# Xiaoming-Zhao/PointNav-VO

Hardware: AMD Instinct MI355X
Metric: RGB-D frame-pair VO inferences/s @341x192 (higher is better)
Workload: dtype f32

## Files before the change

### pointnav-vo_amd/csrc/stem_rs.hip

```cpp
#include <type_traits>

#include "stem_tile.h"

namespace pnvo {

namespace {
constexpr int RS_BUF = XCHG_BYTES;
constexpr int RS_PB_OFF = 2 * RS_BUF;
constexpr int RS_RED_OFF = RS_PB_OFF + 8 * 16 * 33 * 4;
constexpr int RS_ETAB_OFF = RS_RED_OFF + 4 * 2 * 32 * 2 * 4;
constexpr int RS_TRASH_OFF = RS_ETAB_OFF + 64;
constexpr int RS_LDS = RS_TRASH_OFF + 64;
static_assert(RS_BUF >= PATCH_BYTES, "patch must fit its buffer");
static_assert(RS_LDS <= 160 * 1024, "LDS budget");
#define PNVO_INL __attribute__((always_inline))
template <int N, int I = 0, class F>
__device__ __forceinline__ void static_for(F &&f) {
  if constexpr (I < N) {
    f(std::integral_constant<int, I>{});
    static_for<N, I + 1>(f);
  }
}
#ifndef PNVO_RS_LAGD
#define PNVO_RS_LAGD 3
#endif
#ifndef PNVO_RS_LAGP
#define PNVO_RS_LAGP 3
#endif
#ifndef PNVO_RS_GDS
#define PNVO_RS_GDS 2
#endif
#ifndef PNVO_RS_GVM
#define PNVO_RS_GVM 1
#endif
#ifndef PNVO_RS_GVA
#define PNVO_RS_GVA 4
#endif
#ifndef PNVO_RS_A1AHEAD
#define PNVO_RS_A1AHEAD 0
#endif
#ifndef PNVO_RS_MERGE
#define PNVO_RS_MERGE 1
#endif
#ifndef PNVO_RS_MIN_TILES
#define PNVO_RS_MIN_TILES 4
#endif
#ifndef PNVO_RS_NPIN
#define PNVO_RS_NPIN 10
#endif
#ifndef PNVO_RS_ABL
#define PNVO_RS_ABL 0
#endif
}

template <int PIECES, bool POOL, bool RAW, bool FAST = false>
__global__ __launch_bounds__(256) __attribute__((amdgpu_waves_per_eu(1, 1))) void stem_rs_kernel(const StemMXArgs p) {
  static_assert(PIECES == 2 || (PIECES == 1 && !POOL && !FAST), "float16 pieces, or the bf16 dual stem with raw output");
  constexpr bool H = PIECES == 2;
  constexpr int NTL = H ? 1 : 2;
  constexpr int NFT = H ? 5 : 4;
  constexpr bool A1AHEAD = H && PNVO_RS_A1AHEAD;
  constexpr int LAGP = PNVO_RS_LAGP, LAGD = PNVO_RS_LAGD;
  constexpr int GROW = PW * 5;
  extern __shared__ __attribute__((aligned(16))) unsigned char lds[];
  const int tid = threadIdx.x;
  const int lane = tid & 63;
  const int wave = __builtin_amdgcn_readfirstlane(tid >> 6);
  float *red = reinterpret_cast<float *>(lds + RS_RED_OFF);
  float *pb = reinterpret_cast<float *>(lds + RS_PB_OFF);
  float *etab = reinterpret_cast<float *>(lds + RS_ETAB_OFF);

  const int ntiles = p.B * p.tiles_x * p.tiles_y;
  const int chunk = (ntiles + 7) >> 3;
  const int per = (int)gridDim.x >> 3;
  const int t_first = (int)(blockIdx.x & 7) * chunk + (int)(blockIdx.x >> 3);
  const int t_end = min(((int)(blockIdx.x & 7) + 1) * chunk, ntiles);
  if (t_first >= t_end) return;
  const int nit = (t_end - t_first + per - 1) / per;
  const bool prof = p.prof != nullptr;
  unsigned long long pc[4] = {0, 0, 0, 0};
  auto now = [&]() PNVO_INL -> unsigned long long { return prof ? __builtin_readcyclecounter() : 0ull; };
  if (RAW && tid < 12) etab[tid] = p.edges[tid];

  unsigned pmeta[4];
#pragma unroll
  for (int r = 0; r < 4; ++r) {
    const int pix = min(r * 256 + tid, NPIX - 1);
    const int py = pix / PW, px = pix - py * PW;
    pmeta[r] = (unsigned)(py * ROW + (px & 1) * PAR + (px >> 1) * PITCH) | ((unsigned)px << 16) | ((unsigned)py << 22);
  }
  const bool haslast = tid < NPIX - 3 * 256;
  unsigned gm[RAW ? 1 : 3];
  if (!RAW) {
#pragma unroll
    for (int sr = 0; sr < 3; ++sr) {
      const int g = sr * 64 + lane;
      const bool ex = g < GROW;
      const int gg = ex ? g : 0;
      const int px = gg / 5, c = gg - px * 5;
      gm[sr] = (unsigned)((px & 1) * PAR + (px >> 1) * PITCH + c * 8) | ((unsigned)px << 16) | (ex ? 0x80000000u : 0u);
    }
  }
  const unsigned lane16 = (unsigned)lane * 16u;
  const float *zp = p.zero_page;
  const long fpix = (long)p.H * p.W;

  f32x4 vr4[4], gdd[21];
  f32x2 vr2[4], vd[4], vt[4];
  unsigned rgbw[4][2];
  float dv[4][2];
  unsigned pflag[4];
  unsigned lowbits = 0, bad_depth = 0;
  constexpr unsigned OOB = 0x80000000u;
  int shi = 0, swi = 0;
  int st_n = 0, st_ty = 0, st_tx = 0;
  __amdgpu_buffer_rsrc_t r_rgb, r_d, r_dd, r_t;
  auto rsrc = [&](const void *base, long off, long bytes) PNVO_INL {
    return __builtin_amdgcn_make_buffer_rsrc(const_cast<char *>(base ? reinterpret_cast<const char *>(base) + off : reinterpret_cast<const char *>(zp)),
                                             0, base ? (unsigned)bytes : 0u, 0x00020000);
  };
  const int per_n = per / (p.tiles_x * p.tiles_y), per_r = per % (p.tiles_x * p.tiles_y), per_y = per_r / p.tiles_x, per_x = per_r % p.tiles_x;
  auto set_stage_coords = [&](int sn_i, int ty, int tx) PNVO_INL {
    const long sn = sn_i;
    shi = 2 * ty * TH - 3;
    swi = 2 * tx * TW - 3;
    st_n = sn_i;
    st_ty = ty;
    st_tx = tx;
    if (RAW) {
      r_rgb = rsrc(p.raw_rgb, sn * fpix * 6, fpix * 6);
      r_d = rsrc(p.raw_depth, sn * fpix * 8, fpix * 8);
      r_dd = rsrc(nullptr, 0, 0);
    } else {
      r_rgb = rsrc(p.src[0], sn * fpix * 24, fpix * 24);
      r_d = rsrc(p.src[1], sn * fpix * 8, fpix * 8);
      r_dd = rsrc(p.src[2], sn * fpix * 80, fpix * 80);
    }
    r_t = rsrc(p.src[3], sn * fpix * 8, fpix * 8);
  };
  auto stage_next_tile = [&](bool advance) PNVO_INL {
    int tx = st_tx + (advance ? per_x : 0);
    const int cx = tx >= p.tiles_x ? 1 : 0;
    tx -= cx * p.tiles_x;
    int ty = st_ty + (advance ? per_y + cx : 0);
    const int cy = ty >= p.tiles_y ? 1 : 0;
    ty -= cy * p.tiles_y;
    set_stage_coords(st_n + (advance ? per_n + cy : 0), ty, tx);
  };
  auto set_stage_tile = [&](int t) PNVO_INL {
    const int tx = t % p.tiles_x;
    t /= p.tiles_x;
    const int ty = t % p.tiles_y;
    const long sn = t / p.tiles_y;
    shi = 2 * ty * TH - 3;
    swi = 2 * tx * TW - 3;
    st_n = (int)sn;
    st_ty = ty;
    st_tx = tx;
    if (RAW) {
      r_rgb = rsrc(p.raw_rgb, sn * fpix * 6, fpix * 6);
      r_d = rsrc(p.raw_depth, sn * fpix * 8, fpix * 8);
      r_dd = rsrc(nullptr, 0, 0);
    } else {
      r_rgb = rsrc(p.src[0], sn * fpix * 24, fpix * 24);
      r_d = rsrc(p.src[1], sn * fpix * 8, fpix * 8);
      r_dd = rsrc(p.src[2], sn * fpix * 80, fpix * 80);
    }
    r_t = rsrc(p.src[3], sn * fpix * 8, fpix * 8);
  };
  auto opaque = [&](unsigned v) PNVO_INL {
    asm volatile("" : "+v"(v));
    return v;
  };
  auto load_px = [&](int r, bool exists) PNVO_INL {
    const unsigned pm = opaque(pmeta[r]);
    const int hi = shi + (int)(pm >> 22), wi = swi + (int)((pm >> 16) & 0x3fu);
    const bool in = (int)exists & (int)((unsigned)hi < (unsigned)p.H) & (int)((unsigned)wi < (unsigned)p.W);
    const unsigned e = (unsigned)(hi * p.W + wi);
    pflag[r] = (in ? 1u : 0u) | (e > 0u ? 2u : 0u);
    if (RAW) {
#pragma unroll
      for (int f = 0; f < 2; ++f) {
        const unsigned li = (unsigned)f * (unsigned)fpix + e;
        const unsigned boff = 3u * li - ((f > 0 || e > 0u) ? 1u : 0u);
        rgbw[r][f] = __builtin_amdgcn_raw_buffer_load_b32(r_rgb, in ? boff : OOB, 0, 0);
        dv[r][f] = __builtin_bit_cast(float, __builtin_amdgcn_raw_buffer_load_b32(r_d, in ? li * 4u : OOB, 0, 0));
      }
      vt[r] = __builtin_bit_cast(f32x2, __builtin_amdgcn_raw_buffer_load_b64(r_t, in ? e * 8u : OOB, 0, 0));
    } else {
      const unsigned o24 = in ? e * 24u : OOB, o8 = in ? e * 8u : OOB;
      const f32x2 q0 = __builtin_bit_cast(f32x2, __builtin_amdgcn_raw_buffer_load_b64(r_rgb, o24, 0, 0));
      const f32x2 q1 = __builtin_bit_cast(f32x2, __builtin_amdgcn_raw_buffer_load_b64(r_rgb, o24 + 8u, 0, 0));
      vr4[r] = f32x4{q0[0], q0[1], q1[0], q1[1]};
      vr2[r] = __builtin_bit_cast(f32x2, __builtin_amdgcn_raw_buffer_load_b64(r_rgb, o24 + 16u, 0, 0));
      vd[r] = __builtin_bit_cast(f32x2, __builtin_amdgcn_raw_buffer_load_b64(r_d, o8, 0, 0));
      vt[r] = __builtin_bit_cast(f32x2, __builtin_amdgcn_raw_buffer_load_b64(r_t, o8, 0, 0));
    }
  };
  unsigned wrgb[3] = {0u, 0u, 0u};
  constexpr float RGBS = H ? 0.00390625f : 1.f;
  constexpr unsigned ONE2 = H ? 0x3c003c00u : 0x3f803f80u;
  constexpr unsigned short ONE1 = H ? 0x3c00 : 0x3f80;
  auto store_px = [&](int r, unsigned buf, bool exists, int part) PNVO_INL {
    if (part != 2) {
      if (RAW) {
        const unsigned x0 = (pflag[r] & 2u) ? rgbw[r][0] >> 8 : rgbw[r][0], x1 = rgbw[r][1] >> 8;
        const float pr = (float)(x0 & 0xffu), pg = (float)((x0 >> 8) & 0xffu), pbl = (float)((x0 >> 16) & 0xffu);
        const float cr = (float)(x1 & 0xffu), cg = (float)((x1 >> 8) & 0xffu), cb = (float)((x1 >> 16) & 0xffu);
        wrgb[0] = pack_pair<H>(pr * RGBS, pg * RGBS);
        wrgb[1] = pack_pair<H>(pbl * RGBS, cr * RGBS);
        wrgb[2] = pack_pair<H>(cg * RGBS, cb * RGBS);
      } else {
        wrgb[0] = pack_pair<H>(vr4[r][0] * RGBS, vr4[r][1] * RGBS);
        wrgb[1] = pack_pair<H>(vr4[r][2] * RGBS, vr4[r][3] * RGBS);
        wrgb[2] = pack_pair<H>(vr2[r][0] * RGBS, vr2[r][1] * RGBS);
        const float f0 = vr4[r][0], f1 = vr4[r][1], f2 = vr4[r][2], f3 = vr4[r][3], f4 = vr2[r][0], f5 = vr2[r][1];
        lowbits |= __builtin_bit_cast(unsigned, f0) | __builtin_bit_cast(unsigned, f1);
        lowbits |= __builtin_bit_cast(unsigned, f2) | __builtin_bit_cast(unsigned, f3);
        lowbits |= __builtin_bit_cast(unsigned, f4) | __builtin_bit_cast(unsigned, f5);
      }
    }
    if (part == 1) return;
    float d0, d1;
    int bidx[2] = {0, 0};
    unsigned bok[2] = {0u, 0u};
    const bool in = (pflag[r] & 1u) != 0u;
    if (RAW) {
      const bool use_d = (p.raw_flags & 1) != 0;
#pragma unroll
      for (int f = 0; f < 2; ++f) {
        const float d = dv[r][f];
        int g = (int)(d * 10.0f);
        g = min(max(g, 0), 9);
        const float lo = etab[g], hi = etab[g + 1];
        bidx[f] = g - (d < lo ? 1 : 0) + (((d >= hi) & (g < 9)) ? 1 : 0);
        bok[f] = ((d >= 0.f) & (d <= 1.f)) ? 1u : 0u;
        bad_depth |= (pflag[r] & 1u) & (bok[f] ^ 1u);
      }
      d0 = use_d ? dv[r][0] : 0.f;
      d1 = use_d ? dv[r][1] : 0.f;
    } else {
      d0 = vd[r][0];
      d1 = vd[r][1];
    }
    const unsigned w13 = pack_pair<H>(d0, d1), w14 = pack_pair<H>(vt[r][0], vt[r][1]), w15 = in ? ONE2 : 0u;
    const unsigned base = buf + (opaque(pmeta[r]) & 0xffffu);
    constexpr unsigned TR = (unsigned)RS_TRASH_OFF;
    if (RAW) {
      *reinterpret_cast<u32x4 *>(lds + (exists ? base : TR)) = u32x4{0u, 0u, 0u, 0u};
      *reinterpret_cast<u32x4 *>(lds + (exists ? base + 16u : TR)) = u32x4{0u, 0u, 0u, 0u};
      *reinterpret_cast<u32x4 *>(lds + (exists ? base + 32u : TR)) = u32x4{0u, 0u, wrgb[0], wrgb[1]};
      *reinterpret_cast<u32x4 *>(lds + (exists ? base + 48u : TR)) = u32x4{wrgb[2], w13, w14, w15};
      const bool dd = (p.raw_flags & 2) != 0 && in && exists;
      *reinterpret_cast<unsigned short *>(lds + ((dd && bok[0]) ? base + 2u * (unsigned)bidx[0] : TR)) = ONE1;
      *reinterpret_cast<unsigned short *>(lds + ((dd && bok[1]) ? base + 20u + 2u * (unsigned)bidx[1] : TR)) = ONE1;
    } else {
      *reinterpret_cast<u32x2 *>(lds + (exists ? base + 40u : TR)) = u32x2{wrgb[0], wrgb[1]};
      *reinterpret_cast<u32x4 *>(lds + (exists ? base + 48u : TR)) = u32x4{wrgb[2], w13, w14, w15};
    }
    if (H) {
      const f16x2 hd = __builtin_bit_cast(f16x2, w13), ht = __builtin_bit_cast(f16x2, w14);
      const unsigned md = pack_f16(d0 - (float)hd[0], d1 - (float)hd[1]);
      const unsigned mt = pack_f16(vt[r][0] - (float)ht[0], vt[r][1] - (float)ht[1]);
      *reinterpret_cast<u32x4 *>(lds + (exists ? base + 64u : TR)) = u32x4{md, mt, 0u, 0u};
    }
  };
  unsigned ddv[3], ddl[3];
  auto set_dd_tile = [&](unsigned buf) PNVO_INL {
    if (RAW) return;
#pragma unroll
    for (int sr = 0; sr < 3; ++sr) {
      const unsigned g = opaque(gm[sr]);
      const int wi = swi + (int)((g >> 16) & 0x3fu);
      const bool ok = (int)((int)g < 0) & (int)((unsigned)wi < (unsigned)p.W);
      ddv[sr] = ok ? (unsigned)((shi * p.W + swi) * 80 + sr * 1024) + lane16 : OOB;
      ddl[sr] = buf + ((int)g < 0 ? (g & 0xffffu) : (unsigned)(2 * PAR));
    }
  };
  auto load_dd = [&](int slot, int row, int sr) PNVO_INL {
    gdd[slot] = __builtin_bit_cast(f32x4, __builtin_amdgcn_raw_buffer_load_b128(r_dd, ddv[sr] + (unsigned)(row * p.W * 80), 0, 0));
  };
  auto store_dd = [&](int slot, int row, int sr) PNVO_INL {
    const f32x4 v = gdd[slot];
    lowbits |= __builtin_bit_cast(unsigned, v[0]) | __builtin_bit_cast(unsigned, v[1]);
    lowbits |= __builtin_bit_cast(unsigned, v[2]) | __builtin_bit_cast(unsigned, v[3]);
    *reinterpret_cast<u32x2 *>(lds + ddl[sr] + row * ROW) = u32x2{pack_pair<H>(v[0], v[1]), pack_pair<H>(v[2], v[3])};
  };

  const int arr = (lane & 31) >> 4, ac = lane & 15, ah = lane >> 5;
  const unsigned baseA0 = (unsigned)(2 * arr * ROW + ac * PITCH + ah * 16);
  const unsigned baseX0 = (unsigned)(2 * arr * ROW + ac * PITCH + 64);
  const int rr16 = lane >> 5;
  const float oscale = !H ? 1.f : p.oscale_ptr != nullptr ? *p.oscale_ptr : p.oscale;
  const int co = p.y_coff[0] + (lane & 31);
  const float sgn = POOL ? (p.pool_gamma[co] < 0.f ? -1.f : 1.f) : 1.f;

  auto body = [&](auto wv_c) PNVO_INL {
    constexpr int WV = decltype(wv_c)::value;
    constexpr int NROWS = FAST ? (WV == 1 ? 6 : 5) : WV == 3 ? 0 : 7;
    constexpr int DPT = FAST ? 2 : 3, PX0 = FAST ? 1 : 0, PXS = FAST ? 3 : 2;
    auto px_store_tap = [](int i) constexpr { return i >= LAGP + PX0 && (i - LAGP - PX0) % PXS == 0 && (i - LAGP - PX0) / PXS < 3; };
    auto dd_row = [](int j) constexpr { return FAST ? (j < 5 ? WV + 4 * j : 20) : WV + 3 * j; };
    constexpr int RD = RAW ? 0 : 3 * NROWS;
    constexpr int NT = (WV == 3 && !FAST) ? 13 : 12;
    auto tap_of = [](int i) constexpr { return i < 12 ? WV + 4 * i : 48; };
    auto tap_off = [](int t) constexpr { return (t / 7) * ROW + ((t % 7) & 1) * PAR + ((t % 7) >> 1) * PITCH; };

    __syncthreads();
    set_stage_tile(t_first);
    set_dd_tile(0u);
#pragma unroll
    for (int r = 0; r < 3; ++r) load_px(r, true);
    if (WV == 0) load_px(3, haslast);
#pragma unroll
    for (int q = 0; q < RD; ++q) load_dd(q, dd_row(q / 3), q % 3);
#pragma unroll
    for (int r = 0; r < 3; ++r) store_px(r, 0u, true, 0);
    if (WV == 0) store_px(3, 0u, haslast, 0);
#pragma unroll
    for (int q = 0; q < RD; ++q) store_dd(q, dd_row(q / 3), q % 3);
    __syncthreads();

    u32x4 bres[NT][4];
    u32x2 bxr[(H && !FAST) ? NT : 1];
    u32x4 bxs[FAST ? 3 : 1], b48[FAST ? 4 : 1];
    u32x2 b48x = {0u, 0u};
    {
      const u32x4 *wp = reinterpret_cast<const u32x4 *>(p.wpk) + lane;
#pragma unroll
      for (int i = 0; i < NT; ++i) {
#pragma unroll
        for (int f = 0; f < 4; ++f) bres[i][f] = wp[(tap_of(i) * NFT + f) * 64];
        if (H && !FAST) bxr[i] = *reinterpret_cast<const u32x2 *>(wp + (tap_of(i) * NFT + 4) * 64);
      }
      if (FAST) {
        const u32x4 *wq = reinterpret_cast<const u32x4 *>(p.wpk) + (lane & 31);
        const bool kh1 = lane >= 32;
#pragma unroll
        for (int g = 0; g < 3; ++g) {
          const u32x2 lo = *reinterpret_cast<const u32x2 *>(wq + ((kh1 ? tap_of(4 * g + 2) : tap_of(4 * g)) * NFT + 4) * 64);
          const u32x2 hi = *reinterpret_cast<const u32x2 *>(wq + ((kh1 ? tap_of(4 * g + 3) : tap_of(4 * g + 1)) * NFT + 4) * 64);
          bxs[g] = u32x4{lo[0], lo[1], hi[0], hi[1]};
        }
#pragma unroll
        for (int f = 0; f < 4; ++f) b48[f] = wp[(48 * NFT + f) * 64];
        b48x = *reinterpret_cast<const u32x2 *>(wp + (48 * NFT + 4) * 64);
      }
      constexpr int NPIN = H ? PNVO_RS_NPIN : 7;
#pragma unroll
      for (int i = 0; i < (NT < NPIN ? NT : NPIN); ++i) {
#pragma unroll
        for (int f = 0; f < 4; ++f) asm volatile("" : "+a"(bres[i][f]));
        if (H && !FAST) asm volatile("" : "+a"(bxr[i]));
      }
      if (FAST) {
#pragma unroll
        for (int g = 0; g < 3; ++g) asm volatile("" : "+a"(bxs[g]));
      }
    }

    int e_n = 0, e_ho0 = 0, e_wo0 = 0, e_slot = 0;
    bool e_valid = false;
    unsigned ebuf = 0u;
    f32x4 xq[4], tq4;
    float s1 = 0.f, s2 = 0.f, cm[8], pl[6], rs9[3];
    f32x2 rsv[4];
    int rr16v = 0, lc = 0, colv = 0;
    auto epi_begin = [&]() PNVO_INL {
      rr16v = (int)opaque((unsigned)rr16);
      lc = (int)opaque((unsigned)(lane & 31));
      colv = p.Wo - e_wo0 - 4 * rr16v;
      s1 = 0.f;
      s2 = 0.f;
    };
    auto XAl = [&](int rq) PNVO_INL {
#pragma unroll
      for (int s4 = 0; s4 < 4; ++s4)
        xq[s4] = *reinterpret_cast<const f32x4 *>(lds + ebuf + (((WV * 4 + s4) * 4 + rq) * 64 + lane) * 16);
    };
    auto XAs = [&]() PNVO_INL {
#pragma unroll
      for (int e = 0; e < 4; ++e) tq4[e] = (((xq[0][e] + xq[1][e]) + xq[2][e]) + xq[3][e]) * oscale;
    };
    auto XB = [&](int rq) PNVO_INL {
      const bool rowok = e_ho0 + 2 * WV + (rq >> 1) < p.Ho;
#pragma unroll
      for (int e = 0; e < 4; ++e) {
        const int colc = e + 8 * (rq & 1);
        const bool ok = (int)rowok & (int)(colc < colv);
        const float v = ok ? tq4[e] : 0.f;
        pb[((2 * WV + (rq >> 1)) * 16 + colc + 4 * rr16v) * 33 + lc] = ok ? sgn * tq4[e] : -__builtin_inff();
        s1 += v;
        s2 = __builtin_fmaf(v, v, s2);
      }
    };
    auto XC = [&]() PNVO_INL {
      s1 += __shfl_xor(s1, 32);
      s2 += __shfl_xor(s2, 32);
      *reinterpret_cast<f32x2 *>(&red[(WV * 32 + lc) * 2]) = f32x2{s1, s2};
    };
    auto ebar = [&]() PNVO_INL {
      asm volatile("s_waitcnt lgkmcnt(0)\n\ts_barrier" ::: "memory");
    };
    auto PAl = [&](int j) PNVO_INL {
      const int pj = 2 * WV + rr16v;
      const int c0 = pj > 0 ? 2 * pj - 1 : 0, c1 = 2 * pj;
#pragma unroll
      for (int d = 0; d < 2; ++d) {
        pl[3 * d] = pb[((2 * j + d) * 16 + c0) * 33 + lc];
        pl[3 * d + 1] = pb[((2 * j + d) * 16 + c1) * 33 + lc];
        pl[3 * d + 2] = pb[((2 * j + d) * 16 + c1 + 1) * 33 + lc];
      }
    };
    auto PAm = [&](int j) PNVO_INL {
      cm[2 * j] = fmaxf(fmaxf(pl[0], pl[1]), pl[2]);
      cm[2 * j + 1] = fmaxf(fmaxf(pl[3], pl[4]), pl[5]);
    };
    int *e_pool = p.pool;
    unsigned e_joff = 0u, e_j9off = 0u;
    bool e_jok = false, e_j9ok = false;
    auto emit_begin = [&]() PNVO_INL {
      const int pj = 2 * WV + rr16v, J = (e_wo0 >> 1) + pj, J9 = (e_wo0 >> 1) + 8;
      e_pool = p.pool + (long)e_n * p.Hp * p.Wp * p.y_cstride + p.y_coff[0];
      e_joff = (unsigned)(min(J, p.Wp - 1) * p.y_cstride + lc);
      e_j9off = (unsigned)(min(J9, p.Wp - 1) * p.y_cstride + lc);
      e_jok = (int)e_valid & (int)(J < p.Wp);
      e_j9ok = (int)e_valid & (int)(J9 < p.Wp) & (int)(pj < 5);
    };
    auto emit = [&](int I, unsigned joff, float mx, bool valid) PNVO_INL {
      int key = __builtin_bit_cast(int, mx);
      key = key >= 0 ? key : key ^ 0x7fffffff;
      const bool ok = (int)valid & (int)(I < p.Hp);
      atomicMax(e_pool + (long)(min(I, p.Hp - 1) * p.Wp * p.y_cstride) + joff, ok ? key : STEM_POOL_INIT);
    };
    auto PE = [&](int k) PNVO_INL {
      const float mx = k == 0 ? fmaxf(cm[0], cm[1]) : k == 4 ? cm[7] : fmaxf(fmaxf(cm[2 * k - 1], cm[2 * k]), cm[2 * k + 1]);
      emit((e_ho0 >> 1) + k, e_joff, mx, e_jok);
    };
    auto P9l = [&]() PNVO_INL {
      const int pi = 2 * WV + rr16v;
#pragma unroll
      for (int dr = -1; dr <= 1; ++dr) rs9[dr + 1] = pb[(min(max(2 * pi + dr, 0), 7) * 16 + 15) * 33 + lc];
    };
    auto P9e = [&]() PNVO_INL {
      const int pi = 2 * WV + rr16v;
      float mx = -__builtin_inff();
#pragma unroll
      for (int dr = -1; dr <= 1; ++dr) {
        const int lr = 2 * pi + dr;
        mx = fmaxf(mx, ((int)(lr >= 0) & (int)(lr < 8)) ? rs9[dr + 1] : -__builtin_inff());
      }
      emit((e_ho0 >> 1) + pi, e_j9off, mx, e_j9ok);
    };
    auto PSl = [&]() PNVO_INL {
#pragma unroll
      for (int w4 = 0; w4 < 4; ++w4) rsv[w4] = *reinterpret_cast<const f32x2 *>(&red[(w4 * 32 + lc) * 2]);
    };
    auto PSs = [&]() PNVO_INL {
      float a1s = 0.f, a2s = 0.f;
#pragma unroll
      for (int w4 = 0; w4 < 4; ++w4) {
        a1s += rsv[w4][0];
        a2s += rsv[w4][1];
      }
      float *dst = p.stats[0] + (((long)e_n * p.slots + e_slot) * p.stats_cstride + p.y_coff[0]) * 2;
      *reinterpret_cast<f32x2 *>(dst + 2 * lc) = f32x2{a1s, a2s};
    };
    constexpr int ESZ = H ? 4 : 2;
    f32x16 totv[NTL];
    float es1[NTL], es2[NTL];
    __amdgpu_buffer_rsrc_t r_y[NTL];
    unsigned e_yoff = 0u;
    auto out_begin = [&]() PNVO_INL {
#pragma unroll
      for (int nt = 0; nt < NTL; ++nt) {
        const long plane = (long)p.Ho * p.Wo * p.y_cstride * ESZ;
        r_y[nt] = __builtin_amdgcn_make_buffer_rsrc(reinterpret_cast<char *>(p.y[nt]) + (long)e_n * plane + (long)p.y_coff[nt] * ESZ, 0,
                                                    (unsigned)plane, 0x00020000);
        es1[nt] = 0.f;
        es2[nt] = 0.f;
      }
      e_yoff = (unsigned)((((e_ho0 + 2 * WV) * p.Wo + e_wo0 + 4 * rr16v) * p.y_cstride + lc) * ESZ);
    };
    auto XS = [&](int nt, int rq) PNVO_INL {
      const bool rowok = (int)e_valid & (int)(e_ho0 + 2 * WV + (rq >> 1) < p.Ho);
#pragma unroll
      for (int e = 0; e < 4; ++e) {
        const int colc = e + 8 * (rq & 1);
        const bool ok = (int)rowok & (int)(colc < colv);
        const float v = ok ? totv[nt][4 * rq + e] : 0.f;
        const unsigned off = e_yoff + (unsigned)(((rq >> 1) * p.Wo + colc) * p.y_cstride * ESZ);
        if (H)
          __builtin_amdgcn_raw_buffer_store_b32(__builtin_bit_cast(unsigned, v), r_y[nt], ok ? off : OOB, 0, 0);
        else
          __builtin_amdgcn_raw_buffer_store_b16(__builtin_bit_cast(unsigned short, (__bf16)v), r_y[nt], ok ? off : OOB, 0, 0);
        es1[nt] += v;
        es2[nt] = __builtin_fmaf(v, v, es2[nt]);
      }
    };
    auto XCn = [&](int nt) PNVO_INL {
      const float a = es1[nt] + __shfl_xor(es1[nt], 32), b = es2[nt] + __shfl_xor(es2[nt], 32);
      *reinterpret_cast<f32x2 *>(&red[((WV * NTL + nt) * 32 + lc) * 2]) = f32x2{a, b};
    };
    f32x2 rsn[NTL][4];
    auto PSnl = [&](int nt) PNVO_INL {
#pragma unroll
      for (int w4 = 0; w4 < 4; ++w4) rsn[nt][w4] = *reinterpret_cast<const f32x2 *>(&red[((w4 * NTL + nt) * 32 + lc) * 2]);
    };
    auto PSns = [&](int nt) PNVO_INL {
      float a1s = 0.f, a2s = 0.f;
#pragma unroll
      for (int w4 = 0; w4 < 4; ++w4) {
        a1s += rsn[nt][w4][0];
        a2s += rsn[nt][w4][1];
      }
      float *dst = p.stats[nt] + (((long)e_n * p.slots + e_slot) * p.stats_cstride + p.y_coff[nt]) * 2;
      *reinterpret_cast<f32x2 *>(dst + 2 * lc) = f32x2{a1s, a2s};
    };
    auto epi = [&](int i, int rg) PNVO_INL {
      if (PNVO_RS_ABL & 4) return;
      const int k = 5 * i + rg;
      if (!H) {
        const int k4 = 4 * i + rg;
        if (k4 == 0) { epi_begin(); out_begin(); }
        if (k4 == 2) XS(0, 0);
        if (k4 == 3) XS(0, 1);
        if (k4 == 4) XS(0, 2);
        if (k4 == 6) XS(0, 3);
        if (k4 == 7) XS(1, 0);
        if (k4 == 8) XS(1, 1);
        if (k4 == 10) XS(1, 2);
        if (k4 == 11) XS(1, 3);
        if (k4 == 12) { XCn(0); XCn(1); }
        if (k4 == 16 && WV == 1) PSnl(0);
        if (k4 == 16 && WV == 2) PSnl(1);
        if (k4 == 18 && WV == 1) PSns(0);
        if (k4 == 18 && WV == 2) PSns(1);
        return;
      }
      if (!POOL) {
        if (k == 0) { epi_begin(); out_begin(); }
        if (k == 2) XS(0, 0);
        if (k == 3) XS(0, 1);
        if (k == 4) XS(0, 2);
        if (k == 5) XS(0, 3);
        if (k == 7) XCn(0);
        if (k == 15 && WV == 1) PSnl(0);
        if (k == 17 && WV == 1) PSns(0);
        return;
      }
      if (k == 0) epi_begin();
      if ((PNVO_RS_ABL & 8) && k < 15) return;
      if ((PNVO_RS_ABL & 16) && k >= 15) return;
      if (k == 0) XAl(0);
      if (k == 2) { XAs(); XAl(1); }
      if (k == 3) XB(0);
      if (k == 4) { XAs(); XAl(2); }
      if (k == 5) XB(1);
      if (k == 7) { XAs(); XAl(3); }
      if (k == 8) XB(2);
      if (k == 9) XAs();
      if (k == 10) XB(3);
      if (k == 12) XC();
      if (k == 15) PAl(0);
      if (k == 17) { PAm(0); PAl(1); }
      if (k == 20) { PAm(1); PAl(2); }
      if (k == 22) { PAm(2); PAl(3); }
      if (k == 24) { PAm(3); emit_begin(); }
      if (k == 25) PE(0);
      if (k == 27) PE(1);
      if (k == 30) PE(2);
      if (k == 32) PE(3);
      if (k == 35) { PE(4); P9l(); }
      if (k == 37) P9e();
      if (k == 40 && WV == 1) PSl();
      if (k == 42 && WV == 1) PSs();
    };
    auto epi_serial = [&]() PNVO_INL {
      epi_begin();
      if (!POOL) {
        out_begin();
#pragma unroll
        for (int nt = 0; nt < NTL; ++nt) {
#pragma unroll
          for (int rq = 0; rq < 4; ++rq) XS(nt, rq);
          XCn(nt);
        }
        ebar();
        if (WV == 1) {
          PSnl(0);
          PSns(0);
        }
        if (NTL > 1 && WV == 2) {
          PSnl(NTL - 1);
          PSns(NTL - 1);
        }
        return;
      }
#pragma unroll
      for (int rq = 0; rq < 4; ++rq) {
        XAl(rq);
        XAs();
        XB(rq);
      }
      XC();
      ebar();
#pragma unroll
      for (int j = 0; j < 4; ++j) {
        PAl(j);
        PAm(j);
      }
      emit_begin();
#pragma unroll
      for (int k = 0; k < 5; ++k) PE(k);
      P9l();
      P9e();
      if (WV == 1) {
        PSl();
        PSs();
      }
    };

    int c_n = st_n, c_ty = st_ty, c_tx = st_tx;
    e_n = c_n;
    e_ho0 = c_ty * TH;
    e_wo0 = c_tx * TW;
    e_slot = c_ty * p.tiles_x + c_tx;
#pragma unroll 1
    for (int it = 0; it < nit; ++it) {
      const unsigned buf = (unsigned)(it & 1) * RS_BUF, obuf = buf ^ (unsigned)RS_BUF;
      stage_next_tile(it + 1 < nit);
      set_dd_tile(obuf);
      ebuf = obuf;
      const unsigned long long t0 = now();

      f32x16 acc[NTL][4];
      const unsigned baseA = opaque(baseA0 + buf), baseX = opaque(baseX0 + buf);
      u32x4 a0[2][4], a1s[2][4], ax[4];
      u32x4 t48[3];
      const bool xkh = lane >= 32;
      auto tofs = [&](int i, int m) constexpr { return tap_off(tap_of(i)) + m * 4 * ROW; };
#pragma unroll
      for (int m = 0; m < 4; ++m) {
        a0[0][m] = *reinterpret_cast<const u32x4 *>(lds + baseA + tofs(0, m));
        if (A1AHEAD) a1s[0][m] = *reinterpret_cast<const u32x4 *>(lds + baseA + tofs(0, m) + 32);
      }
      auto region_end = [&](bool hard = true) PNVO_INL {
#pragma unroll
        for (int k = 0; k < 4; ++k) {
          __builtin_amdgcn_sched_group_barrier(0x008, 1, 0);
          __builtin_amdgcn_sched_group_barrier(0x100, PNVO_RS_GDS, 0);
          __builtin_amdgcn_sched_group_barrier(0x010, PNVO_RS_GVM, 0);
          __builtin_amdgcn_sched_group_barrier(0x002, PNVO_RS_GVA, 0);
          __builtin_amdgcn_sched_group_barrier(0x200, 1, 0);
        }
        if (hard) __builtin_amdgcn_sched_barrier(0);
      };
      auto mfma4 = [&](const u32x4 *aq, const u32x4 bq, bool first = false, int nt = 0) PNVO_INL {
        const f32x16 zero = {0.f, 0.f, 0.f, 0.f, 0.f, 0.f, 0.f, 0.f, 0.f, 0.f, 0.f, 0.f, 0.f, 0.f, 0.f, 0.f};
#pragma unroll
        for (int m = 0; m < 4; ++m)
          acc[nt][m] = H ? __builtin_amdgcn_mfma_f32_32x32x16_f16(__builtin_bit_cast(f16x8, aq[m]), __builtin_bit_cast(f16x8, bq),
                                                                  first ? zero : acc[nt][m], 0, 0, 0)
                         : __builtin_amdgcn_mfma_f32_32x32x16_bf16(__builtin_bit_cast(bf16x8, aq[m]), __builtin_bit_cast(bf16x8, bq),
                                                                   first ? zero : acc[nt][m], 0, 0, 0);
      };
      __builtin_amdgcn_sched_barrier(0);
      static_for<NT>([&](auto ic) PNVO_INL {
        constexpr int i = decltype(ic)::value;
        const bool st = !(PNVO_RS_ABL & 2), sd = !RAW && !(PNVO_RS_ABL & 1);
        if (H) {
#pragma unroll
          for (int m = 0; m < 4; ++m) {
            if (!A1AHEAD) a1s[i & 1][m] = *reinterpret_cast<const u32x4 *>(lds + baseA + tofs(i, m) + 32);
            if (!FAST) ax[m] = *reinterpret_cast<const u32x4 *>(lds + baseX + tofs(i, m));
          }
          if (FAST && i > 0 && (i - 1) % 4 != 3) {
            epi(i - 1, 4);
            if (st && px_store_tap(i - 1)) store_px((i - 1 - LAGP - PX0) / PXS, obuf, true, 2);
          }
          epi(i, 0);
          mfma4(a0[i & 1], bres[i][0], i == 0);
          region_end(!(PNVO_RS_MERGE & 1));
          if (sd) {
#pragma unroll
            for (int q = DPT * i; q < DPT * i + DPT; ++q)
              if (q < RD) load_dd(q, dd_row(q / 3), q % 3);
          }
          if (st && i >= PX0 && (i - PX0) % PXS == 0 && (i - PX0) / PXS < 3) load_px((i - PX0) / PXS, true);
          if (st && WV == 0 && i == 8) load_px(3, haslast);
          mfma4(a0[i & 1], bres[i][2]);
          region_end(!(PNVO_RS_MERGE & 2));
          if (i + 1 < NT) {
#pragma unroll
            for (int m = 0; m < 4; ++m) a0[(i + 1) & 1][m] = *reinterpret_cast<const u32x4 *>(lds + baseA + tofs(i + 1, m));
          }
          if (FAST && i % 4 == 3) {
            const unsigned xa = baseX + (unsigned)(xkh ? tofs(i - 1, 0) : tofs(i - 3, 0)), xb = baseX + (unsigned)(xkh ? tofs(i, 0) : tofs(i - 2, 0));
#pragma unroll
            for (int m = 0; m < 4; ++m) {
              const u32x2 lo = *reinterpret_cast<const u32x2 *>(lds + xa + m * 4 * ROW), hi = *reinterpret_cast<const u32x2 *>(lds + xb + m * 4 * ROW);
              ax[m] = u32x4{lo[0], lo[1], hi[0], hi[1]};
            }
          }
          if (FAST && i == 11) {
            t48[0] = *reinterpret_cast<const u32x4 *>(lds + baseA + tap_off(48) + WV * 4 * ROW);
            t48[1] = *reinterpret_cast<const u32x4 *>(lds + baseA + tap_off(48) + WV * 4 * ROW + 32);
            t48[2] = *reinterpret_cast<const u32x4 *>(lds + baseX + tap_off(48) + WV * 4 * ROW);
          }
          epi(i, 2);
          mfma4(a1s[i & 1], bres[i][1]);
          region_end(!(PNVO_RS_MERGE & 1));
          if (sd && i >= LAGD) {
#pragma unroll
            for (int q = DPT * (i - LAGD); q < DPT * (i - LAGD) + DPT; ++q)
              if (q < RD) store_dd(q, dd_row(q / 3), q % 3);
          }
          if (st && px_store_tap(i)) store_px((i - LAGP - PX0) / PXS, obuf, true, 1);
          if (A1AHEAD && i + 1 < NT) {
#pragma unroll
            for (int m = 0; m < 4; ++m) a1s[(i + 1) & 1][m] = *reinterpret_cast<const u32x4 *>(lds + baseA + tofs(i + 1, m) + 32);
          }
          epi(i, 3);
          mfma4(a1s[i & 1], bres[i][3]);
          region_end(!(PNVO_RS_MERGE & 4));
          if (!FAST || i % 4 == 3) {
            if (st && px_store_tap(i)) store_px((i - LAGP - PX0) / PXS, obuf, true, 2);
            if (st && WV == 0 && i == 11) store_px(3, obuf, haslast, 0);
            epi(i, 4);
            mfma4(ax, FAST ? bxs[FAST ? i / 4 : 0] : u32x4{bxr[FAST ? 0 : i][0], bxr[FAST ? 0 : i][1], 0u, 0u});
            region_end();
          }
          if (FAST && i == 11) {
            const u32x4 bq5[5] = {b48[0], b48[2], b48[1], b48[3], u32x4{b48x[0], b48x[1], 0u, 0u}};
#pragma unroll
            for (int g5 = 0; g5 < 5; ++g5)
              acc[0][WV] = __builtin_amdgcn_mfma_f32_32x32x16_f16(__builtin_bit_cast(f16x8, t48[g5 < 2 ? 0 : g5 < 4 ? 1 : 2]),
                                                                  __builtin_bit_cast(f16x8, bq5[g5]), acc[0][WV], 0, 0, 0);
            __builtin_amdgcn_sched_barrier(0);
          }
        } else {
#pragma unroll
          for (int m = 0; m < 4; ++m) a1s[i & 1][m] = *reinterpret_cast<const u32x4 *>(lds + baseA + tofs(i, m) + 32);
          epi(i, 0);
          mfma4(a0[i & 1], bres[i][0], i == 0, 0);
          region_end(!(PNVO_RS_MERGE & 1));
          if (sd) {
#pragma unroll
            for (int q = 3 * i; q < 3 * i + 3; ++q)
              if (q < RD) load_dd(q, dd_row(q / 3), q % 3);
          }
          if (st && i % 2 == 0 && i < 6) load_px(i / 2, true);
          if (st && WV == 0 && i == 8) load_px(3, haslast);
          mfma4(a0[i & 1], bres[i][1], i == 0, 1);
          region_end();
          if (i + 1 < NT) {
#pragma unroll
            for (int m = 0; m < 4; ++m) a0[(i + 1) & 1][m] = *reinterpret_cast<const u32x4 *>(lds + baseA + tofs(i + 1, m));
          }
          if (st && i >= LAGP + 1 && (i - LAGP - 1) % 2 == 0 && i - LAGP - 1 < 6) store_px((i - LAGP - 1) / 2, obuf, true, 2);
          if (st && WV == 0 && i == 11) store_px(3, obuf, haslast, 0);
          epi(i, 2);
          mfma4(a1s[i & 1], bres[i][2], false, 0);
          region_end(!(PNVO_RS_MERGE & 1));
          if (sd && i >= LAGD) {
#pragma unroll
            for (int q = 3 * (i - LAGD); q < 3 * (i - LAGD) + 3; ++q)
              if (q < RD) store_dd(q, dd_row(q / 3), q % 3);
          }
          if (st && i >= LAGP && (i - LAGP) % 2 == 0 && i - LAGP < 6) store_px((i - LAGP) / 2, obuf, true, 1);
          epi(i, 3);
          mfma4(a1s[i & 1], bres[i][3], false, 1);
          region_end();
        }
        if (i == (H ? 2 : 3) && !(PNVO_RS_ABL & 32)) ebar();
      });
      const unsigned long long t1 = now();
      __syncthreads();
      const unsigned long long t2 = now();
      const int n = c_n, ty = c_ty, tx = c_tx;
      if (POOL) {
#pragma unroll
        for (int m = 0; m < 4; ++m)
#pragma unroll
          for (int rq = 0; rq < 4; ++rq)
            *reinterpret_cast<f32x4 *>(lds + buf + (((m * 4 + WV) * 4 + rq) * 64 + lane) * 16) =
                f32x4{acc[0][m][4 * rq], acc[0][m][4 * rq + 1], acc[0][m][4 * rq + 2], acc[0][m][4 * rq + 3]};
        __syncthreads();
        e_n = n;
        e_ho0 = ty * TH;
        e_wo0 = tx * TW;
        e_slot = ty * p.tiles_x + tx;
        e_valid = true;
      } else {
#pragma unroll
        for (int nt = 0; nt < NTL; ++nt) {
          if (nt > 0) __syncthreads();
#pragma unroll
          for (int m = 0; m < 4; ++m)
#pragma unroll
            for (int rq = 0; rq < 4; ++rq)
              *reinterpret_cast<f32x4 *>(lds + buf + (((m * 4 + WV) * 4 + rq) * 64 + lane) * 16) =
                  f32x4{acc[nt][m][4 * rq], acc[nt][m][4 * rq + 1], acc[nt][m][4 * rq + 2], acc[nt][m][4 * rq + 3]};
          __syncthreads();
#pragma unroll
          for (int s4 = 0; s4 < 4; ++s4)
#pragma unroll
            for (int rq = 0; rq < 4; ++rq) {
              const f32x4 tq = *reinterpret_cast<const f32x4 *>(lds + buf + (((WV * 4 + s4) * 4 + rq) * 64 + lane) * 16);
#pragma unroll
              for (int e = 0; e < 4; ++e) totv[nt][4 * rq + e] = s4 == 0 ? tq[e] : totv[nt][4 * rq + e] + tq[e];
            }
          if (H) {
#pragma unroll
            for (int r = 0; r < 16; ++r) totv[nt][r] *= oscale;
          }
        }
        e_n = n;
        e_ho0 = ty * TH;
        e_wo0 = tx * TW;
        e_slot = ty * p.tiles_x + tx;
        e_valid = true;
      }
      c_n = st_n;
      c_ty = st_ty;
      c_tx = st_tx;
      if (prof) {
        pc[0] += t1 - t0;
        pc[1] += t2 - t1;
        pc[2] += now() - t2;
      }
    }
    ebuf = (unsigned)((nit - 1) & 1) * RS_BUF;
    epi_serial();
  };
  switch (wave) {
    case 0: body(std::integral_constant<int, 0>{}); break;
    case 1: body(std::integral_constant<int, 1>{}); break;
    case 2: body(std::integral_constant<int, 2>{}); break;
    default: body(std::integral_constant<int, 3>{}); break;
  }
  if (H && !RAW && (lowbits & 0x1fffu) != 0 && p.bad_input != nullptr) *p.bad_input = 1;
  if (RAW && bad_depth != 0u && p.raw_err != nullptr) *p.raw_err = 1;
  if (prof && lane == 0 && (blockIdx.x % 16) == 0) {
    unsigned long long *q = p.prof + 16 * wave;
#pragma unroll
    for (int k = 0; k < 3; ++k) atomicAdd(q + k, pc[k]);
    atomicAdd(q + 5, (unsigned long long)nit);
  }
}

bool stem_rs_takes(const StemMXArgs &a, int pieces, int ntiles_n, bool bf16_out, int wgs) {
  const long ntiles = (long)a.B * ((a.Wo + TW - 1) / TW) * ((a.Ho + TH - 1) / TH);
  const bool f16 = pieces == 2 && ntiles_n == 1 && !bf16_out, dual = pieces == 1 && ntiles_n == 2 && bf16_out && a.pool == nullptr;
  return (f16 || dual) && wgs >= 8 && ntiles >= PNVO_RS_MIN_TILES * (long)wgs;
}

hipError_t launch_stem_rs(const StemMXArgs &a, int pieces, bool fast, int wgs, hipStream_t s) {
  static std::mutex attr_mu;
  static unsigned long long attr_seen = 0;
  if (pnvo_first_launch_on_device(attr_mu, attr_seen)) {
    hipError_t e = hipSuccess;
    auto set = [&](const void *f) {
      if (e == hipSuccess) e = hipFuncSetAttribute(f, hipFuncAttributeMaxDynamicSharedMemorySize, RS_LDS);
    };
    set(reinterpret_cast<const void *>(stem_rs_kernel<2, true, true>));
    set(reinterpret_cast<const void *>(stem_rs_kernel<2, true, false>));
    set(reinterpret_cast<const void *>(stem_rs_kernel<2, false, true>));
    set(reinterpret_cast<const void *>(stem_rs_kernel<2, false, false>));
    set(reinterpret_cast<const void *>(stem_rs_kernel<2, true, true, true>));
    set(reinterpret_cast<const void *>(stem_rs_kernel<2, true, false, true>));
    set(reinterpret_cast<const void *>(stem_rs_kernel<2, false, true, true>));
    set(reinterpret_cast<const void *>(stem_rs_kernel<2, false, false, true>));
    set(reinterpret_cast<const void *>(stem_rs_kernel<1, false, true>));
    set(reinterpret_cast<const void *>(stem_rs_kernel<1, false, false>));
    if (e != hipSuccess) return e;
  }
  StemMXArgs p = a;
  p.tiles_x = (a.Wo + TW - 1) / TW;
  p.tiles_y = (a.Ho + TH - 1) / TH;
  const dim3 g((unsigned)(wgs & ~7)), b(256);
  const bool raw = p.raw_depth != nullptr, pool = p.pool != nullptr;
#define PNVO_RS_LAUNCH(...) hipLaunchKernelGGL((stem_rs_kernel<__VA_ARGS__>), g, b, RS_LDS, s, p)
  if (pieces == 1) {
    if (raw) PNVO_RS_LAUNCH(1, false, true);
    else PNVO_RS_LAUNCH(1, false, false);
  } else if (fast) {
    if (pool && raw) PNVO_RS_LAUNCH(2, true, true, true);
    else if (pool) PNVO_RS_LAUNCH(2, true, false, true);
    else if (raw) PNVO_RS_LAUNCH(2, false, true, true);
    else PNVO_RS_LAUNCH(2, false, false, true);
  } else {
    if (pool && raw) PNVO_RS_LAUNCH(2, true, true);
    else if (pool) PNVO_RS_LAUNCH(2, true, false);
    else if (raw) PNVO_RS_LAUNCH(2, false, true);
    else PNVO_RS_LAUNCH(2, false, false);
  }
#undef PNVO_RS_LAUNCH
  return hipGetLastError();
}

}
```

Before: 112,300.

## Overlap final tap-48 MFMAs with accumulator LDS exchange stores

The five tap-48 MFMAs that closed the last iteration of the FAST tap loop now run after the barrier, interleaved with the LDS stores of the other wavefronts' accumulator blocks. The wave's own block is stored last, once its accumulation is complete. Buffer resource construction is simplified to precomputed bases and sizes with a 32-bit per-sample offset, and the pooling sign is folded into the scale multiplier. Stage-tile setup is moved after the initial A-operand LDS loads behind a sched_barrier. The aim is to hide MFMA latency behind exchange stores and cut scalar address math, at the cost of a more intricate epilogue ordering.

```diff
diff --git a/pointnav-vo_amd/csrc/stem_rs.hip b/pointnav-vo_amd/csrc/stem_rs.hip
--- a/pointnav-vo_amd/csrc/stem_rs.hip
+++ b/pointnav-vo_amd/csrc/stem_rs.hip
@@ -115,28 +115,27 @@
   int shi = 0, swi = 0;
   int st_n = 0, st_ty = 0, st_tx = 0;
   __amdgpu_buffer_rsrc_t r_rgb, r_d, r_dd, r_t;
-  auto rsrc = [&](const void *base, long off, long bytes) PNVO_INL {
-    return __builtin_amdgcn_make_buffer_rsrc(const_cast<char *>(base ? reinterpret_cast<const char *>(base) + off : reinterpret_cast<const char *>(zp)),
-                                             0, base ? (unsigned)bytes : 0u, 0x00020000);
+  auto in_base = [&](const void *base) PNVO_INL { return base ? reinterpret_cast<const char *>(base) : reinterpret_cast<const char *>(zp); };
+  auto in_bytes = [&](const void *base, long bytes) PNVO_INL { return base ? (unsigned)bytes : 0u; };
+  const char *b_rgb = in_base(RAW ? (const void *)p.raw_rgb : (const void *)p.src[0]), *b_d = in_base(RAW ? (const void *)p.raw_depth : (const void *)p.src[1]);
+  const char *b_dd = in_base(RAW ? nullptr : p.src[2]), *b_t = in_base(p.src[3]);
+  const unsigned n_rgb = in_bytes(RAW ? (const void *)p.raw_rgb : (const void *)p.src[0], RAW ? fpix * 6 : fpix * 24);
+  const unsigned n_d = in_bytes(RAW ? (const void *)p.raw_depth : (const void *)p.src[1], fpix * 8);
+  const unsigned n_dd = in_bytes(RAW ? nullptr : p.src[2], fpix * 80), n_t = in_bytes(p.src[3], fpix * 8);
+  auto rsrc = [&](const char *base, unsigned bytes, int sn) PNVO_INL {
+    return __builtin_amdgcn_make_buffer_rsrc(const_cast<char *>(base + (unsigned long)(unsigned)sn * bytes), 0, bytes, 0x00020000);
   };
   const int per_n = per / (p.tiles_x * p.tiles_y), per_r = per % (p.tiles_x * p.tiles_y), per_y = per_r / p.tiles_x, per_x = per_r % p.tiles_x;
-  auto set_stage_coords = [&](int sn_i, int ty, int tx) PNVO_INL {
-    const long sn = sn_i;
+  auto set_stage_coords = [&](int sn, int ty, int tx) PNVO_INL {
     shi = 2 * ty * TH - 3;
     swi = 2 * tx * TW - 3;
-    st_n = sn_i;
+    st_n = sn;
     st_ty = ty;
     st_tx = tx;
-    if (RAW) {
-      r_rgb = rsrc(p.raw_rgb, sn * fpix * 6, fpix * 6);
-      r_d = rsrc(p.raw_depth, sn * fpix * 8, fpix * 8);
-      r_dd = rsrc(nullptr, 0, 0);
-    } else {
-      r_rgb = rsrc(p.src[0], sn * fpix * 24, fpix * 24);
-      r_d = rsrc(p.src[1], sn * fpix * 8, fpix * 8);
-      r_dd = rsrc(p.src[2], sn * fpix * 80, fpix * 80);
-    }
-    r_t = rsrc(p.src[3], sn * fpix * 8, fpix * 8);
+    r_rgb = rsrc(b_rgb, n_rgb, sn);
+    r_d = rsrc(b_d, n_d, sn);
+    r_dd = rsrc(b_dd, n_dd, sn);
+    r_t = rsrc(b_t, n_t, sn);
   };
   auto stage_next_tile = [&](bool advance) PNVO_INL {
     int tx = st_tx + (advance ? per_x : 0);
@@ -151,22 +150,7 @@
     const int tx = t % p.tiles_x;
     t /= p.tiles_x;
     const int ty = t % p.tiles_y;
-    const long sn = t / p.tiles_y;
-    shi = 2 * ty * TH - 3;
-    swi = 2 * tx * TW - 3;
-    st_n = (int)sn;
-    st_ty = ty;
-    st_tx = tx;
-    if (RAW) {
-      r_rgb = rsrc(p.raw_rgb, sn * fpix * 6, fpix * 6);
-      r_d = rsrc(p.raw_depth, sn * fpix * 8, fpix * 8);
-      r_dd = rsrc(nullptr, 0, 0);
-    } else {
-      r_rgb = rsrc(p.src[0], sn * fpix * 24, fpix * 24);
-      r_d = rsrc(p.src[1], sn * fpix * 8, fpix * 8);
-      r_dd = rsrc(p.src[2], sn * fpix * 80, fpix * 80);
-    }
-    r_t = rsrc(p.src[3], sn * fpix * 8, fpix * 8);
+    set_stage_coords(t / p.tiles_y, ty, tx);
   };
   auto opaque = [&](unsigned v) PNVO_INL {
     asm volatile("" : "+v"(v));
@@ -294,6 +278,7 @@
   const float oscale = !H ? 1.f : p.oscale_ptr != nullptr ? *p.oscale_ptr : p.oscale;
   const int co = p.y_coff[0] + (lane & 31);
   const float sgn = POOL ? (p.pool_gamma[co] < 0.f ? -1.f : 1.f) : 1.f;
+  const float osg = oscale * sgn;
 
   auto body = [&](auto wv_c) PNVO_INL {
     constexpr int WV = decltype(wv_c)::value;
@@ -380,7 +365,7 @@
     };
     auto XAs = [&]() PNVO_INL {
 #pragma unroll
-      for (int e = 0; e < 4; ++e) tq4[e] = (((xq[0][e] + xq[1][e]) + xq[2][e]) + xq[3][e]) * oscale;
+      for (int e = 0; e < 4; ++e) tq4[e] = (((xq[0][e] + xq[1][e]) + xq[2][e]) + xq[3][e]) * osg;
     };
     auto XB = [&](int rq) PNVO_INL {
       const bool rowok = e_ho0 + 2 * WV + (rq >> 1) < p.Ho;
@@ -389,7 +374,7 @@
         const int colc = e + 8 * (rq & 1);
         const bool ok = (int)rowok & (int)(colc < colv);
         const float v = ok ? tq4[e] : 0.f;
-        pb[((2 * WV + (rq >> 1)) * 16 + colc + 4 * rr16v) * 33 + lc] = ok ? sgn * tq4[e] : -__builtin_inff();
+        pb[((2 * WV + (rq >> 1)) * 16 + colc + 4 * rr16v) * 33 + lc] = ok ? tq4[e] : -__builtin_inff();
         s1 += v;
         s2 = __builtin_fmaf(v, v, s2);
       }
@@ -397,7 +382,7 @@
     auto XC = [&]() PNVO_INL {
       s1 += __shfl_xor(s1, 32);
       s2 += __shfl_xor(s2, 32);
-      *reinterpret_cast<f32x2 *>(&red[(WV * 32 + lc) * 2]) = f32x2{s1, s2};
+      *reinterpret_cast<f32x2 *>(&red[(WV * 32 + lc) * 2]) = f32x2{sgn * s1, s2};
     };
     auto ebar = [&]() PNVO_INL {
       asm volatile("s_waitcnt lgkmcnt(0)\n\ts_barrier" ::: "memory");
@@ -629,11 +614,6 @@
 #pragma unroll 1
     for (int it = 0; it < nit; ++it) {
       const unsigned buf = (unsigned)(it & 1) * RS_BUF, obuf = buf ^ (unsigned)RS_BUF;
-      stage_next_tile(it + 1 < nit);
-      set_dd_tile(obuf);
-      ebuf = obuf;
-      const unsigned long long t0 = now();
-
       f32x16 acc[NTL][4];
       const unsigned baseA = opaque(baseA0 + buf), baseX = opaque(baseX0 + buf);
       u32x4 a0[2][4], a1s[2][4], ax[4];
@@ -645,6 +625,12 @@
         a0[0][m] = *reinterpret_cast<const u32x4 *>(lds + baseA + tofs(0, m));
         if (A1AHEAD) a1s[0][m] = *reinterpret_cast<const u32x4 *>(lds + baseA + tofs(0, m) + 32);
       }
+      __builtin_amdgcn_sched_barrier(0);
+      stage_next_tile(it + 1 < nit);
+      set_dd_tile(obuf);
+      ebuf = obuf;
+      const unsigned long long t0 = now();
+
       auto region_end = [&](bool hard = true) PNVO_INL {
 #pragma unroll
         for (int k = 0; k < 4; ++k) {
@@ -731,14 +717,6 @@
             mfma4(ax, FAST ? bxs[FAST ? i / 4 : 0] : u32x4{bxr[FAST ? 0 : i][0], bxr[FAST ? 0 : i][1], 0u, 0u});
             region_end();
           }
-          if (FAST && i == 11) {
-            const u32x4 bq5[5] = {b48[0], b48[2], b48[1], b48[3], u32x4{b48x[0], b48x[1], 0u, 0u}};
-#pragma unroll
-            for (int g5 = 0; g5 < 5; ++g5)
-              acc[0][WV] = __builtin_amdgcn_mfma_f32_32x32x16_f16(__builtin_bit_cast(f16x8, t48[g5 < 2 ? 0 : g5 < 4 ? 1 : 2]),
-                                                                  __builtin_bit_cast(f16x8, bq5[g5]), acc[0][WV], 0, 0, 0);
-            __builtin_amdgcn_sched_barrier(0);
-          }
         } else {
 #pragma unroll
           for (int m = 0; m < 4; ++m) a1s[i & 1][m] = *reinterpret_cast<const u32x4 *>(lds + baseA + tofs(i, m) + 32);
@@ -779,13 +757,29 @@
       __syncthreads();
       const unsigned long long t2 = now();
       const int n = c_n, ty = c_ty, tx = c_tx;
+      auto xstore = [&](int nt, int m) PNVO_INL {
+#pragma unroll
+        for (int rq = 0; rq < 4; ++rq)
+          *reinterpret_cast<f32x4 *>(lds + buf + (((m * 4 + WV) * 4 + rq) * 64 + lane) * 16) =
+              f32x4{acc[nt][m][4 * rq], acc[nt][m][4 * rq + 1], acc[nt][m][4 * rq + 2], acc[nt][m][4 * rq + 3]};
+      };
+      auto xchg = [&](int nt) PNVO_INL {
+        if constexpr (FAST) {
+          const u32x4 bq5[5] = {b48[0], b48[2], b48[1], b48[3], u32x4{b48x[0], b48x[1], 0u, 0u}};
+#pragma unroll
+          for (int g5 = 0; g5 < 5; ++g5) {
+            if (g5 < 3) xstore(nt, (WV + 1 + g5) & 3);
+            acc[0][WV] = __builtin_amdgcn_mfma_f32_32x32x16_f16(__builtin_bit_cast(f16x8, t48[g5 < 2 ? 0 : g5 < 4 ? 1 : 2]),
+                                                                __builtin_bit_cast(f16x8, bq5[g5]), acc[0][WV], 0, 0, 0);
+          }
+          xstore(nt, WV);
+        } else {
+#pragma unroll
+          for (int m = 0; m < 4; ++m) xstore(nt, m);
+        }
+      };
       if (POOL) {
-#pragma unroll
-        for (int m = 0; m < 4; ++m)
-#pragma unroll
-          for (int rq = 0; rq < 4; ++rq)
-            *reinterpret_cast<f32x4 *>(lds + buf + (((m * 4 + WV) * 4 + rq) * 64 + lane) * 16) =
-                f32x4{acc[0][m][4 * rq], acc[0][m][4 * rq + 1], acc[0][m][4 * rq + 2], acc[0][m][4 * rq + 3]};
+        xchg(0);
         __syncthreads();
         e_n = n;
         e_ho0 = ty * TH;
@@ -796,12 +790,7 @@
 #pragma unroll
         for (int nt = 0; nt < NTL; ++nt) {
           if (nt > 0) __syncthreads();
-#pragma unroll
-          for (int m = 0; m < 4; ++m)
-#pragma unroll
-            for (int rq = 0; rq < 4; ++rq)
-              *reinterpret_cast<f32x4 *>(lds + buf + (((m * 4 + WV) * 4 + rq) * 64 + lane) * 16) =
-                  f32x4{acc[nt][m][4 * rq], acc[nt][m][4 * rq + 1], acc[nt][m][4 * rq + 2], acc[nt][m][4 * rq + 3]};
+          xchg(nt);
           __syncthreads();
 #pragma unroll
           for (int s4 = 0; s4 < 4; ++s4)
```

New measurement: 112,300, median of 6. About the same (+0.0%).
